# near/near-light-client

Hardware: AMD Instinct MI355X
Metric: Sync/Verify proofs/sec at 1/2/4/8 MI355X + achieved HBM GB/s vs roofline (higher is better)
Workload: dtype u64 (Goldilocks field, integer)

## Files before the change

### near-light-client_amd/csrc/gl32.hpp

```cpp
#pragma once
#include "gl.hpp"
#include "poseidon_blocks.inc"

namespace gl32 {

struct F {
    uint32_t lo, hi;
};

__device__ __forceinline__ F from_u64(uint64_t x) { return F{(uint32_t)x, (uint32_t)(x >> 32)}; }
__device__ __forceinline__ uint64_t to_u64(F x) { return ((uint64_t)x.hi << 32) | x.lo; }

__device__ __forceinline__ F add_w2_eps(uint64_t base, uint32_t w2) {
    uint64_t r;
    uint32_t t;
    asm("v_mad_u64_u32 %[r], vcc, %[w2], -1, %[base]\n\t"
        "v_cndmask_b32_e64 %[t], 0, -1, vcc\n\t"
        "v_mad_u64_u32 %[r], vcc, %[t], 1, %[r]"
        : [r] "=&v"(r), [t] "=&v"(t)
        : [w2] "v"(w2), [base] "v"(base)
        : "vcc");
    return from_u64(r);
}

__device__ __forceinline__ F reduce128(uint32_t w0, uint32_t w1, uint32_t w2, uint32_t w3) {
    uint32_t r0, r1, t0;
    asm("v_sub_co_u32 %[r0], vcc, %[w0], %[w3]\n\t"
        "v_subbrev_co_u32 %[r1], vcc, 0, %[w1], vcc\n\t"
        "v_cndmask_b32_e64 %[t0], 0, -1, vcc\n\t"
        "v_sub_co_u32 %[r0], vcc, %[r0], %[t0]\n\t"
        "v_subbrev_co_u32 %[r1], vcc, 0, %[r1], vcc"
        : [r0] "=&v"(r0), [r1] "=&v"(r1), [t0] "=&v"(t0)
        : [w0] "v"(w0), [w1] "v"(w1), [w3] "v"(w3)
        : "vcc");
    return add_w2_eps(((uint64_t)r1 << 32) | r0, w2);
}

__device__ __forceinline__ uint64_t mad_u64_one(uint32_t a, uint64_t c);

__device__ __forceinline__ F mul(F a, F b) {
#ifdef NLX_GL32_MUL_CARRY_CHAINS
    uint64_t t = (uint64_t)a.lo * b.lo;
    uint64_t m = (uint64_t)a.lo * b.hi;
    uint64_t x = (uint64_t)a.hi * b.hi;
    uint64_t mid;
    uint32_t x1;
    asm("v_mad_u64_u32 %[mid], vcc, %[ah], %[bl], %[m]\n\t"
        "v_addc_co_u32 %[x1], vcc, 0, %[xh], vcc"
        : [mid] "=&v"(mid), [x1] "=v"(x1)
        : [ah] "v"(a.hi), [bl] "v"(b.lo), [m] "v"(m), [xh] "v"((uint32_t)(x >> 32))
        : "vcc");
    uint32_t r0, r1, w1, w2, w3, t0;
    asm("v_add_co_u32 %[w1], vcc, %[th], %[m0]\n\t"
        "v_addc_co_u32 %[w2], vcc, %[x0], %[m1], vcc\n\t"
        "v_addc_co_u32 %[w3], vcc, 0, %[x1], vcc\n\t"
        "v_sub_co_u32 %[r0], vcc, %[w0], %[w3]\n\t"
        "v_subbrev_co_u32 %[r1], vcc, 0, %[w1], vcc\n\t"
        "v_cndmask_b32_e64 %[t0], 0, -1, vcc\n\t"
        "v_sub_co_u32 %[r0], vcc, %[r0], %[t0]\n\t"
        "v_subbrev_co_u32 %[r1], vcc, 0, %[r1], vcc"
        : [r0] "=&v"(r0), [r1] "=&v"(r1), [w1] "=&v"(w1), [w2] "=&v"(w2), [w3] "=&v"(w3), [t0] "=&v"(t0)
        : [w0] "v"((uint32_t)t), [th] "v"((uint32_t)(t >> 32)), [m0] "v"((uint32_t)mid), [x0] "v"((uint32_t)x),
          [m1] "v"((uint32_t)(mid >> 32)), [x1] "v"(x1)
        : "vcc");
    return add_w2_eps(((uint64_t)r1 << 32) | r0, w2);
#else
    const uint64_t p0 = (uint64_t)a.lo * b.lo;
    const uint64_t p1 = (uint64_t)a.lo * b.hi + (p0 >> 32);
    const uint64_t p2 = (uint64_t)a.hi * b.lo + (uint32_t)p1;
    uint64_t p3 = (uint64_t)a.hi * b.hi + (p1 >> 32);
    p3 = mad_u64_one((uint32_t)(p2 >> 32), p3);
    return reduce128((uint32_t)p0, (uint32_t)p2, (uint32_t)p3, (uint32_t)(p3 >> 32));
#endif
}

__device__ __forceinline__ F add_const(F a, uint64_t c) {
    F r;
    uint32_t t;
    asm("v_add_co_u32 %[r0], vcc, %[a0], %[c0]\n\t"
        "v_addc_co_u32 %[r1], vcc, %[a1], %[c1], vcc\n\t"
        "v_cndmask_b32_e64 %[t], 0, -1, vcc\n\t"
        "v_add_co_u32 %[r0], vcc, %[r0], %[t]\n\t"
        "v_addc_co_u32 %[r1], vcc, 0, %[r1], vcc"
        : [r0] "=&v"(r.lo), [r1] "=&v"(r.hi), [t] "=&v"(t)
        : [a0] "v"(a.lo), [a1] "v"(a.hi), [c0] "s"((uint32_t)c), [c1] "v"((uint32_t)(c >> 32))
        : "vcc");
    return r;
}

__device__ __forceinline__ F add_const_v(F a, uint64_t c) {
    F r;
    uint32_t t;
    asm("v_add_co_u32 %[r0], vcc, %[a0], %[c0]\n\t"
        "v_addc_co_u32 %[r1], vcc, %[a1], %[c1], vcc\n\t"
        "v_cndmask_b32_e64 %[t], 0, -1, vcc\n\t"
        "v_add_co_u32 %[r0], vcc, %[r0], %[t]\n\t"
        "v_addc_co_u32 %[r1], vcc, 0, %[r1], vcc"
        : [r0] "=&v"(r.lo), [r1] "=&v"(r.hi), [t] "=&v"(t)
        : [a0] "v"(a.lo), [a1] "v"(a.hi), [c0] "v"((uint32_t)c), [c1] "v"((uint32_t)(c >> 32))
        : "vcc");
    return r;
}

__device__ __forceinline__ F sbox7(F x) {
    F x2 = mul(x, x);
    F x4 = mul(x2, x2);
    F x3 = mul(x, x2);
    return mul(x3, x4);
}

__device__ __forceinline__ F fold_acc(uint64_t al, uint64_t ah) {
    uint64_t t;
    asm("v_mad_u64_u32 %[t], vcc, %[ah1], -1, %[al]" : [t] "=&v"(t) : [ah1] "v"((uint32_t)(ah >> 32)), [al] "v"(al) : "vcc");
    uint32_t r1, m;
    asm("v_add_co_u32 %[r1], vcc, %[t1], %[ah0]\n\t"
        "v_cndmask_b32_e64 %[m], 0, -1, vcc"
        : [r1] "=v"(r1), [m] "=v"(m)
        : [t1] "v"((uint32_t)(t >> 32)), [ah0] "v"((uint32_t)ah)
        : "vcc");
    uint64_t r;
    asm("v_mad_u64_u32 %[r], vcc, %[m], 1, %[base]" : [r] "=&v"(r) : [m] "v"(m), [base] "v"(((uint64_t)r1 << 32) | (uint32_t)t) : "vcc");
    return from_u64(r);
}

__device__ __forceinline__ void mds_layer(F (&s)[12], const uint64_t* __restrict__ rc_next = nullptr) {
    constexpr uint32_t C[12] = {17, 15, 41, 16, 2, 28, 13, 13, 39, 18, 34, 20};
    F o[12];
#pragma unroll
    for (int r = 0; r < 12; r++) {
        uint64_t al = 0, ah = 0;
        if (rc_next) {
            const uint64_t c = rc_next[r];
            al = (uint32_t)c;
            ah = c >> 32;
        }
#pragma unroll
        for (int i = 0; i < 12; i++) {
            al += (uint64_t)s[(i + r) % 12].lo * C[i];
            ah += (uint64_t)s[(i + r) % 12].hi * C[i];
        }
        if (r == 0) {
            al += (uint64_t)s[0].lo * 8u;
            ah += (uint64_t)s[0].hi * 8u;
        }
        o[r] = fold_acc(al, ah);
    }
#pragma unroll
    for (int i = 0; i < 12; i++) s[i] = o[i];
}


typedef int i32x4_t __attribute__((ext_vector_type(4)));
typedef int i32x16_t __attribute__((ext_vector_type(16)));

__device__ __forceinline__ void keep_whole(const i32x16_t& d) { asm volatile("" : : "v"(d)); }

__device__ __forceinline__ i32x4_t mds_a_fragment(uint32_t lane = threadIdx.x & 63) {
    constexpr int C[12] = {17, 15, 41, 16, 2, 28, 13, 13, 39, 18, 34, 20};
    const uint32_t rho = lane & 31, h = lane >> 5;
    const uint32_t g = (rho >> 2) & 1, r = (rho & 3) + 4 * (rho >> 3);
    uint32_t w[4] = {0, 0, 0, 0};
    if (h == g && rho < 24) {
#pragma unroll
        for (int j = 0; j < 12; j++) {
            uint32_t m = 0;
#pragma unroll
            for (int rr = 0; rr < 12; rr++)
                if ((uint32_t)rr == r) m = (uint32_t)C[(j - rr + 12) % 12] + ((rr == 0 && j == 0) ? 8u : 0u);
            w[j >> 2] |= m << (8 * (j & 3));
        }
        w[3] = r == 0 ? 0x00F88080u : 0x00008080u;
    }
    i32x4_t a;
    a.x = (int)w[0]; a.y = (int)w[1]; a.z = (int)w[2]; a.w = (int)w[3];
    return a;
}
constexpr uint32_t MDS_B_BIAS_SLOTS = 0x00808080u;

__device__ __forceinline__ void transpose_bytes4(uint32_t x0, uint32_t x1, uint32_t x2, uint32_t x3, uint32_t (&p)[4]) {
    const uint32_t t01l = __builtin_amdgcn_perm(x1, x0, 0x05010400u), t01h = __builtin_amdgcn_perm(x1, x0, 0x07030602u);
    const uint32_t t23l = __builtin_amdgcn_perm(x3, x2, 0x05010400u), t23h = __builtin_amdgcn_perm(x3, x2, 0x07030602u);
    p[0] = __builtin_amdgcn_perm(t23l, t01l, 0x05040100u);
    p[1] = __builtin_amdgcn_perm(t23l, t01l, 0x07060302u);
    p[2] = __builtin_amdgcn_perm(t23h, t01h, 0x05040100u);
    p[3] = __builtin_amdgcn_perm(t23h, t01h, 0x07060302u);
}
__device__ __forceinline__ uint64_t mad_u64(uint32_t a, uint32_t b, uint64_t c) {
    uint64_t r, sink;
    asm("v_mad_u64_u32 %0, %1, %2, %3, %4" : "=v"(r), "=s"(sink) : "v"(a), "v"(b), "v"(c));
    return r;
}
__device__ __forceinline__ uint64_t mad_u64_sc(uint32_t a, uint32_t b, uint64_t c_uniform) {
    uint64_t r, sink;
    asm("v_mad_u64_u32 %0, %1, %2, %3, %4" : "=v"(r), "=s"(sink) : "v"(a), "v"(b), "s"(c_uniform));
    return r;
}
__device__ __forceinline__ uint64_t mad_u64_one(uint32_t a, uint64_t c) {
    uint64_t r, sink;
    asm("v_mad_u64_u32 %0, %1, %2, 1, %3" : "=v"(r), "=s"(sink) : "v"(a), "v"(c));
    return r;
}
__device__ __forceinline__ F fold_pair(uint64_t t, uint32_t yh, uint32_t k16) {
    uint64_t z, u, sink, sink2;
    asm("v_mad_u64_u32 %0, %1, %2, %3, 0" : "=v"(z), "=s"(sink) : "v"(yh), "v"(k16));
    asm("v_mad_u64_u32 %0, %1, %2, -1, %3" : "=v"(u), "=s"(sink2) : "v"((uint32_t)(z >> 32)), "v"(t));
    uint32_t r1, m;
    asm("v_add_co_u32 %0, vcc, %2, %3\n\t"
        "v_cndmask_b32_e64 %1, 0, -1, vcc"
        : "=v"(r1), "=v"(m)
        : "v"((uint32_t)(u >> 32)), "v"((uint32_t)z)
        : "vcc");
    return from_u64(mad_u64_one(m, ((uint64_t)r1 << 32) | (uint32_t)u));
}

template <int RC>
__device__ __forceinline__ void mds_layer_mfma(F (&s)[12], const i32x4_t a, const uint64_t* __restrict__ rcb) {
    uint32_t k16 = 65536u, bw = MDS_B_BIAS_SLOTS;
    asm("" : "+v"(k16));
    asm("" : "+v"(bw));
    i32x16_t zero;
#pragma unroll
    for (int i = 0; i < 16; i++) zero[i] = 0;
    uint32_t x[2][12], y[2][12];
#pragma unroll
    for (int half = 0; half < 2; half++) {
        uint32_t pl[4][3];
#pragma unroll
        for (int q = 0; q < 3; q++) {
            uint32_t p[4];
            if (half == 0)
                transpose_bytes4(s[4 * q].lo ^ 0x80808080u, s[4 * q + 1].lo ^ 0x80808080u, s[4 * q + 2].lo ^ 0x80808080u,
                                 s[4 * q + 3].lo ^ 0x80808080u, p);
            else
                transpose_bytes4(s[4 * q].hi ^ 0x80808080u, s[4 * q + 1].hi ^ 0x80808080u, s[4 * q + 2].hi ^ 0x80808080u,
                                 s[4 * q + 3].hi ^ 0x80808080u, p);
#pragma unroll
            for (int b = 0; b < 4; b++) pl[b][q] = p[b];
        }
        i32x16_t d[4];
#pragma unroll
        for (int b = 0; b < 4; b++) {
            i32x4_t bf;
            bf.x = (int)pl[b][0]; bf.y = (int)pl[b][1]; bf.z = (int)pl[b][2]; bf.w = (int)bw;
            d[b] = __builtin_amdgcn_mfma_i32_32x32x32_i8(a, bf, zero, 0, 0, 0);
        }
#pragma unroll
        for (int b = 0; b < 4; b++) keep_whole(d[b]);
#pragma unroll
        for (int r = 0; r < 12; r++) {
            x[half][r] = ((uint32_t)d[1][r] << 8) + (uint32_t)d[0][r];
            y[half][r] = ((uint32_t)d[3][r] << 8) + (uint32_t)d[2][r];
        }
        __builtin_amdgcn_sched_barrier(0);
    }
#pragma unroll
    for (int r = 0; r < 12; r++) {
        if (RC == 2 || (RC == 1 && r == 0)) {
            const uint64_t al = mad_u64_one(x[0][r], mad_u64_sc(y[0][r], k16, rcb[r]));
            const uint64_t ah = mad_u64_one(x[1][r], mad_u64_sc(y[1][r], k16, rcb[12 + r]));
            s[r] = fold_acc(al, ah);
        } else {
            const uint64_t t = mad_u64(y[0][r], k16, ((uint64_t)x[1][r] << 32) | x[0][r]);
            s[r] = fold_pair(t, y[1][r], k16);
        }
    }
}

struct BlockOperands {
    i32x4_t a[3];
    i32x16_t seed;
};

template <int G>
__device__ __forceinline__ uint64_t mad_u64_imm(uint32_t a, uint64_t c) {
    uint64_t r, sink;
    asm("v_mad_u64_u32 %0, %1, %2, %3, %4" : "=v"(r), "=s"(sink) : "v"(a), "n"(G), "v"(c));
    return r;
}
__device__ __forceinline__ F fold_pair_x(uint64_t t, uint32_t yh, uint32_t x2, uint32_t k16) {
    uint64_t z, u, sink, sink2;
    asm("v_mad_u64_u32 %0, %1, %2, %3, 0" : "=v"(z), "=s"(sink) : "v"(yh), "v"(k16));
    const uint32_t e = (uint32_t)(z >> 32) + x2;
    asm("v_mad_u64_u32 %0, %1, %2, -1, %3" : "=v"(u), "=s"(sink2) : "v"(e), "v"(t));
    uint32_t r1, m;
    asm("v_add_co_u32 %0, vcc, %2, %3\n\t"
        "v_cndmask_b32_e64 %1, 0, -1, vcc"
        : "=v"(r1), "=v"(m)
        : "v"((uint32_t)(u >> 32)), "v"((uint32_t)z)
        : "vcc");
    return from_u64(mad_u64_one(m, ((uint64_t)r1 << 32) | (uint32_t)u));
}
__device__ __forceinline__ uint64_t mad_u64_sm(uint32_t a, uint32_t m_uniform, uint64_t c) {
    uint64_t r, sink;
    asm("v_mad_u64_u32 %0, %1, %2, %3, %4" : "=v"(r), "=s"(sink) : "v"(a), "s"(m_uniform), "v"(c));
    return r;
}
template <typename RHO>
__device__ __forceinline__ void dot12(const F (&z)[12], const RHO& rho, uint64_t klo, uint64_t khi, uint64_t& al, uint64_t& ah) {
    al = klo;
    ah = khi;
#pragma unroll
    for (int j = 0; j < 12; j++) {
        al = mad_u64_sm(z[j].lo, rho.v[j], al);
        ah = mad_u64_sm(z[j].hi, rho.v[j], ah);
    }
}
struct BlockRho1 { static constexpr uint32_t v[12] = NLX_POSEIDON_BLOCK_RHO1_INIT; };
struct BlockRho2 { static constexpr uint32_t v[12] = NLX_POSEIDON_BLOCK_RHO2_INIT; };

struct BlockSboxes {
    __device__ __forceinline__ F first(F s0) const { return sbox7(s0); }
    __device__ __forceinline__ F inner(int, F w) const { return sbox7(w); }
    __device__ __forceinline__ void before_matrix_pass() const {}
};

template <int GAMMA21, class Sboxes = BlockSboxes>
__device__ __forceinline__ void partial_block3(F (&s)[12], const BlockOperands& op, const uint64_t* __restrict__ kap,
                                               Sboxes sb = Sboxes{}) {
    uint32_t k16 = 65536u;
    asm("" : "+v"(k16));
    s[0] = sb.first(s[0]);
    uint64_t al, ah;
    dot12(s, BlockRho1{}, kap[2], kap[3], al, ah);
    const F u1 = sb.inner(1, fold_acc(al, ah));
    dot12(s, BlockRho2{}, kap[4], kap[5], al, ah);
    al = mad_u64_imm<GAMMA21>(u1.lo, al);
    ah = mad_u64_imm<GAMMA21>(u1.hi, ah);
    const F u2 = sb.inner(2, fold_acc(al, ah));
    sb.before_matrix_pass();
    uint32_t pl[8][3];
#pragma unroll
    for (int half = 0; half < 2; half++)
#pragma unroll
        for (int q = 0; q < 3; q++) {
            uint32_t p[4];
            if (half == 0)
                transpose_bytes4(s[4 * q].lo ^ 0x80808080u, s[4 * q + 1].lo ^ 0x80808080u, s[4 * q + 2].lo ^ 0x80808080u,
                                 s[4 * q + 3].lo ^ 0x80808080u, p);
            else
                transpose_bytes4(s[4 * q].hi ^ 0x80808080u, s[4 * q + 1].hi ^ 0x80808080u, s[4 * q + 2].hi ^ 0x80808080u,
                                 s[4 * q + 3].hi ^ 0x80808080u, p);
#pragma unroll
            for (int b = 0; b < 4; b++) pl[4 * half + b][q] = p[b];
        }
    uint32_t w3[8];
    {
// ... 57 lines not shown
```

### near-light-client_amd/csrc/hash_kernels.hip

```cpp
#include <hip/hip_runtime.h>
#include "poseidon.hpp"
#include "launch.hpp"

namespace nlx {

__global__ __launch_bounds__(256, 4) void k_permute_batch(uint64_t* __restrict__ states, size_t n) {
    const size_t t_raw = (size_t)blockIdx.x * blockDim.x + threadIdx.x;
    const bool live = t_raw < n;
    const size_t t = live ? t_raw : n - 1;
    uint64_t s[12];
    const ulonglong2* src = reinterpret_cast<const ulonglong2*>(states + t * 12);
#pragma unroll
    for (int i = 0; i < 6; i++) {
        ulonglong2 v = src[i];
        s[2 * i] = v.x;
        s[2 * i + 1] = v.y;
    }
    poseidon::permute(s);
    if (!live) return;
    ulonglong2* dst = reinterpret_cast<ulonglong2*>(states + t * 12);
#pragma unroll
    for (int i = 0; i < 6; i++) dst[i] = make_ulonglong2(s[2 * i], s[2 * i + 1]);
}

__device__ __forceinline__ void store_digest(uint64_t* __restrict__ out, size_t idx, const uint64_t (&s)[12]) {
    ulonglong2* dst = reinterpret_cast<ulonglong2*>(out + idx * 4);
    dst[0] = make_ulonglong2(gl::canon(s[0]), gl::canon(s[1]));
    dst[1] = make_ulonglong2(gl::canon(s[2]), gl::canon(s[3]));
}

__global__ __launch_bounds__(256, 4) void k_hash_leaves_rowmajor(const uint64_t* __restrict__ rows, uint32_t row_len,
                                                              size_t n_rows, uint64_t* __restrict__ digests) {
    const size_t row_raw = (size_t)blockIdx.x * blockDim.x + threadIdx.x;
    const bool live = row_raw < n_rows;
    const size_t row = live ? row_raw : n_rows - 1;
    uint64_t s[12];
#pragma unroll
    for (int i = 0; i < 12; i++) s[i] = 0;
    const uint64_t* p = rows + row * (size_t)row_len;
    if (row_len <= 4) {
        for (uint32_t c = 0; c < row_len; c++) {
            uint64_t v = p[c];
            if (c == 0) s[0] = v; else if (c == 1) s[1] = v; else if (c == 2) s[2] = v; else s[3] = v;
        }
        if (live) store_digest(digests, row, s);
        return;
    }
#pragma unroll 1
    for (uint32_t c = 0; c < row_len; c += 8) {
        const uint32_t rem = row_len - c;
#pragma unroll
        for (int j = 0; j < 8; j++)
            if ((uint32_t)j < rem) s[j] = p[c + j];
        poseidon::permute_loose(s);
    }
    if (live) store_digest(digests, row, s);
}

__global__ __launch_bounds__(256, 4) void k_merkle_level(const uint64_t* __restrict__ children,
                                                      uint64_t* __restrict__ parents, size_t n_parents, size_t tree_words) {
    children += (size_t)blockIdx.y * tree_words;
    parents += (size_t)blockIdx.y * tree_words;
    const size_t i_raw = (size_t)blockIdx.x * blockDim.x + threadIdx.x;
    const bool live = i_raw < n_parents;
    const size_t i = live ? i_raw : n_parents - 1;
    const ulonglong2* src = reinterpret_cast<const ulonglong2*>(children + i * 8);
    uint64_t s[12];
#pragma unroll
    for (int k = 0; k < 4; k++) {
        ulonglong2 v = src[k];
        s[2 * k] = v.x;
        s[2 * k + 1] = v.y;
    }
    s[8] = s[9] = s[10] = s[11] = 0;
    poseidon::permute_loose(s);
    if (live) store_digest(parents, i, s);
}

constexpr size_t MERKLE_WIDE_MAX_PARENTS = (size_t)1 << 14;
constexpr unsigned MERKLE_FUSED_MAX_LEVELS = 6;
void launch_merkle_fused(hipStream_t st, const uint64_t* children, size_t n_children, unsigned levels, uint32_t n_trees, size_t tree_words);

void launch_permute_batch(hipStream_t st, uint64_t* d_states, size_t n) {
    if (!n) return;
    hipLaunchKernelGGL(k_permute_batch, dim3((unsigned)((n + 255) / 256)), dim3(256), 0, st, d_states, n);
}

void launch_hash_leaves_rowmajor(hipStream_t st, const uint64_t* d_rows, uint32_t row_len, size_t n_rows,
                                 uint64_t* d_digests) {
    if (!n_rows) return;
    hipLaunchKernelGGL(k_hash_leaves_rowmajor, dim3((unsigned)((n_rows + 255) / 256)), dim3(256), 0, st, d_rows,
                       row_len, n_rows, d_digests);
}

const uint64_t* launch_merkle_levels(hipStream_t st, uint64_t* d_digests, size_t n_leaves, unsigned cap_height, uint32_t n_trees, size_t tree_words) {
    size_t cap = (size_t)1 << cap_height;
    uint64_t* cur = d_digests;
    size_t lvl = n_leaves;
    while (lvl > cap) {
        uint64_t* nxt = cur + lvl * 4;
        size_t half = lvl >> 1;
        if (half <= MERKLE_WIDE_MAX_PARENTS) {
            unsigned K = 0;
            while (K < MERKLE_FUSED_MAX_LEVELS && (lvl >> K) > cap) K++;
            launch_merkle_fused(st, cur, lvl, K, n_trees, tree_words);
            for (unsigned s = 0; s < K; s++) {
                cur += lvl * 4;
                lvl >>= 1;
            }
            continue;
        }
        hipLaunchKernelGGL(k_merkle_level, dim3((unsigned)((half + 255) / 256), n_trees), dim3(256), 0, st, cur, nxt, half, tree_words);
        cur = nxt;
        lvl = half;
    }
    return cur;
}

}

namespace nlx {

constexpr size_t HASH_LEAVES_WIDE_MAX_ROWS = (size_t)1 << 13;

__global__ __launch_bounds__(256, 4) void k_hash_lde_leaves(const uint64_t* __restrict__ lde, size_t col_stride,
                                                         uint32_t n_cols, unsigned log_n, unsigned rate_bits,
                                                         uint64_t* __restrict__ digests, uint32_t batch_cols, size_t tree_words) {
    if (batch_cols) {
        const uint32_t c0 = blockIdx.y * batch_cols;
        lde += (size_t)c0 * col_stride;
        n_cols = n_cols - c0 < batch_cols ? n_cols - c0 : batch_cols;
        digests += (size_t)blockIdx.y * tree_words;
    }
    const size_t pos_raw = (size_t)blockIdx.x * blockDim.x + threadIdx.x;
    const bool live = (pos_raw >> (log_n + rate_bits)) == 0;
    const size_t pos = live ? pos_raw : ((size_t)1 << (log_n + rate_bits)) - 1;
    uint64_t s[12];
#pragma unroll
    for (int i = 0; i < 12; i++) s[i] = 0;
    const uint64_t* p = lde + pos;
    const uint32_t r = (uint32_t)(pos >> log_n), k = (uint32_t)(pos & (((size_t)1 << log_n) - 1));
    const size_t leaf = ((size_t)gl::bitrev32(r, rate_bits) << log_n) + gl::bitrev32(k, log_n);
    if (n_cols <= 4) {
        for (uint32_t c = 0; c < n_cols; c++) {
            uint64_t v = p[(size_t)c * col_stride];
            if (c == 0) s[0] = v; else if (c == 1) s[1] = v; else if (c == 2) s[2] = v; else s[3] = v;
        }
        if (live) store_digest(digests, leaf, s);
        return;
    }
#pragma unroll 1
    for (uint32_t c = 0; c < n_cols; c += 8) {
        const uint32_t rem = n_cols - c;
#pragma unroll
        for (int j = 0; j < 8; j++)
            if ((uint32_t)j < rem) s[j] = p[(size_t)(c + j) * col_stride];
        poseidon::permute_loose(s);
    }
    if (live) store_digest(digests, leaf, s);
}

void launch_hash_lde_leaves_wide(hipStream_t st, const uint64_t* d_lde, size_t col_stride, uint32_t n_cols, unsigned log_n,
                                 unsigned rate_bits, uint64_t* d_digests, uint32_t batch_cols, size_t tree_words);

__global__ __launch_bounds__(256, 4) void k_hash_lde_groups(const uint64_t* __restrict__ lde, size_t col_stride, uint32_t n_cols,
                                                            uint32_t group, unsigned log_L, uint64_t* __restrict__ out) {
    const size_t pos_raw = (size_t)blockIdx.x * blockDim.x + threadIdx.x;
    const bool live = (pos_raw >> log_L) == 0;
    const size_t L = (size_t)1 << log_L, pos = live ? pos_raw : L - 1;
    const uint32_t g = blockIdx.y, c0 = g * group, c1 = c0 + group < n_cols ? c0 + group : n_cols;
    uint64_t s[12];
#pragma unroll
    for (int i = 0; i < 12; i++) s[i] = 0;
    const uint64_t* p = lde + pos;
#pragma unroll 1
    for (uint32_t c = c0; c < c1; c += 8) {
        const uint32_t rem = c1 - c;
#pragma unroll
        for (int j = 0; j < 8; j++)
            if ((uint32_t)j < rem) s[j] = p[(size_t)(c + j) * col_stride];
        poseidon::permute_loose(s);
    }
    if (!live) return;
#pragma unroll
    for (int j = 0; j < 4; j++) out[((size_t)(4 * g + j) << log_L) + pos] = gl::canon(s[j]);
}

void launch_hash_lde_leaves_grouped(hipStream_t st, const uint64_t* d_lde, size_t col_stride, uint32_t n_cols, uint32_t group,
                                    unsigned log_n, unsigned rate_bits, uint64_t* d_group_digests, uint64_t* d_digests) {
    const size_t rows = (size_t)1 << (log_n + rate_bits);
    const uint32_t K = (n_cols + group - 1) / group;
    hipLaunchKernelGGL(k_hash_lde_groups, dim3((unsigned)((rows + 255) / 256), K), dim3(256), 0, st, d_lde, col_stride, n_cols, group,
                       log_n + rate_bits, d_group_digests);
    launch_hash_lde_leaves(st, d_group_digests, rows, 4 * K, log_n, rate_bits, d_digests, 0, 0);
}

void launch_hash_lde_leaves(hipStream_t st, const uint64_t* d_lde, size_t col_stride, uint32_t n_cols,
                            unsigned log_n, unsigned rate_bits, uint64_t* d_digests, uint32_t batch_cols, size_t tree_words) {
    size_t rows = (size_t)1 << (log_n + rate_bits);
    const uint32_t n_batches = batch_cols ? (n_cols + batch_cols - 1) / batch_cols : 1;
    const uint32_t widest = batch_cols && batch_cols < n_cols ? batch_cols : n_cols;
    if (rows * n_batches <= HASH_LEAVES_WIDE_MAX_ROWS && widest > 16) {
        launch_hash_lde_leaves_wide(st, d_lde, col_stride, n_cols, log_n, rate_bits, d_digests, batch_cols, tree_words);
        return;
    }
    hipLaunchKernelGGL(k_hash_lde_leaves, dim3((unsigned)((rows + 255) / 256), n_batches), dim3(256), 0, st, d_lde, col_stride,
                       n_cols, log_n, rate_bits, d_digests, batch_cols, tree_words);
}

}

namespace nlx {

constexpr unsigned WIDE_GROUPS_PER_BLOCK = 16;

__device__ __forceinline__ gl32::F permute_wide(gl32::F x, uint32_t j, volatile uint64_t* slot) {
    constexpr uint32_t C[12] = {17, 15, 41, 16, 2, 28, 13, 13, 39, 18, 34, 20};
    const uint64_t* rc = poseidon::RC_DEV;
    const uint32_t jj = j < 12 ? j : 0;
    const uint32_t diag = j == 0 ? 8u : 0u;
#pragma unroll 1
    for (int r = 0; r < 30; r++) {
        x = gl32::add_const_v(x, rc[r * 12 + jj]);
        const gl32::F x7 = gl32::sbox7(x);
        const bool full = (r < 4) || (r >= 26);
        if (full || j == 0) x = x7;
        volatile uint64_t* sl = slot + (r & 1) * 12;
        if (j < 12) sl[j] = gl32::to_u64(x);
        __builtin_amdgcn_fence(__ATOMIC_RELEASE, "wavefront");
        __builtin_amdgcn_wave_barrier();
        __builtin_amdgcn_fence(__ATOMIC_ACQUIRE, "wavefront");
        uint64_t al = (uint64_t)x.lo * diag, ah = (uint64_t)x.hi * diag, bl = 0, bh = 0;
#pragma unroll
        for (int i = 0; i < 12; i += 2) {
            uint32_t s0 = jj + i, s1 = jj + i + 1;
            s0 = s0 >= 12 ? s0 - 12 : s0;
            s1 = s1 >= 12 ? s1 - 12 : s1;
            const uint64_t v0 = sl[s0], v1 = sl[s1];
            al += (uint64_t)(uint32_t)v0 * C[i];
            ah += (uint64_t)(uint32_t)(v0 >> 32) * C[i];
            bl += (uint64_t)(uint32_t)v1 * C[i + 1];
            bh += (uint64_t)(uint32_t)(v1 >> 32) * C[i + 1];
        }
        x = gl32::fold_acc(al + bl, ah + bh);
    }
    return x;
}

constexpr unsigned FUSED_GROUPS = 32;

__global__ __launch_bounds__(FUSED_GROUPS * 16) void k_merkle_fused(const uint64_t* __restrict__ children, uint64_t* __restrict__ parents0,
                                                                   size_t n_children, unsigned K, size_t tree_words) {
    children += (size_t)blockIdx.y * tree_words;
    parents0 += (size_t)blockIdx.y * tree_words;
    __shared__ uint64_t slots[FUSED_GROUPS * 24];
    __shared__ uint64_t lv[2][FUSED_GROUPS * 2 * 4];
    const uint32_t j = threadIdx.x & 15, g = threadIdx.x >> 4;
    const uint32_t n_own = 1u << K;
    for (uint32_t i = threadIdx.x; i < n_own * 4; i += FUSED_GROUPS * 16) lv[0][i] = children[((size_t)blockIdx.x << K) * 4 + i];
    __syncthreads();
    uint64_t* outp = parents0;
    size_t level_total = n_children;
    for (unsigned s = 1; s <= K; s++) {
        const uint32_t own = n_own >> s;
// ... 101 lines not shown
```

### near-light-client_amd/csrc/poseidon.hpp

```cpp
#pragma once
#include "gl.hpp"
#if defined(__HIP__)
#include "gl32.hpp"
#endif
#include "poseidon_constants.inc"

namespace poseidon {

constexpr int WIDTH = 12;
constexpr int RATE = 8;
constexpr int N_ROUNDS = 30;
constexpr int HALF_FULL = 4;
constexpr int N_PARTIAL = 22;

#if defined(__HIP__)
__constant__ static const uint64_t RC_DEV[360] = NLX_POSEIDON_ROUND_CONSTANTS_INIT;
__constant__ static const uint64_t LAYER_RCB_DEV[31 * 24] = NLX_POSEIDON_LAYER_RCB_INIT;
__constant__ static const uint32_t BLOCK_FRAGMENTS_DEV[NLX_POSEIDON_BLOCK_K * 64 * 4] = NLX_POSEIDON_BLOCK_FRAGMENTS_INIT;
__constant__ static const uint32_t BLOCK_SEED_DEV[16] = NLX_POSEIDON_BLOCK_SEED_INIT;
__constant__ static const uint64_t BLOCK_KAPPA_DEV[NLX_POSEIDON_N_BLOCKS * 2 * NLX_POSEIDON_BLOCK_K] = NLX_POSEIDON_BLOCK_KAPPA_INIT;
static_assert(NLX_POSEIDON_BLOCK_K == 3 && NLX_POSEIDON_BLOCK_DMAX < (1 << 20), "gl32::partial_block3 is written for these");

__device__ __forceinline__ gl32::BlockOperands block_operands(uint32_t lane = threadIdx.x & 63) {
    gl32::BlockOperands op;
#pragma unroll
    for (int p = 0; p < 3; p++) {
        const uint32_t* f = BLOCK_FRAGMENTS_DEV + (p * 64 + lane) * 4;
        op.a[p].x = (int)f[0]; op.a[p].y = (int)f[1]; op.a[p].z = (int)f[2]; op.a[p].w = (int)f[3];
    }
    const uint32_t zero = lane >> 6;
#pragma unroll
    for (int i = 0; i < 16; i++) op.seed[i] = (int)(BLOCK_SEED_DEV[i] + zero);
    return op;
}
#endif
static const uint64_t RC_HOST[360] = NLX_POSEIDON_ROUND_CONSTANTS_INIT;

GL_HD const uint64_t* rc_table() {
#if defined(__HIP_DEVICE_COMPILE__)
    return RC_DEV;
#else
    return RC_HOST;
#endif
}

GL_HD uint64_t sbox7(uint64_t x) {
    uint64_t x2 = gl::mul_loose(x, x);
    uint64_t x4 = gl::mul_loose(x2, x2);
    uint64_t x3 = gl::mul_loose(x, x2);
    return gl::mul_loose(x3, x4);
}

GL_HD uint64_t mds_fold(uint64_t al, uint64_t ah) {
    uint64_t l = al + (ah << 32);
    uint64_t h = (ah >> 32) + (l < al ? 1u : 0u);
    uint64_t t1 = (h << 32) - h;
    uint64_t res = l + t1;
    if (res < t1) res += gl::EPS;
    return res;
}
GL_HD void mds_layer(uint64_t (&s)[12]) {
    constexpr uint32_t C[12] = {17, 15, 41, 16, 2, 28, 13, 13, 39, 18, 34, 20};
    uint32_t lo[12], hi[12];
#pragma unroll
    for (int i = 0; i < 12; i++) {
        lo[i] = (uint32_t)s[i];
        hi[i] = (uint32_t)(s[i] >> 32);
    }
#pragma unroll
    for (int r = 0; r < 12; r++) {
        uint64_t al = 0, ah = 0;
#pragma unroll
        for (int i = 0; i < 12; i++) {
            al += (uint64_t)lo[(i + r) % 12] * C[i];
            ah += (uint64_t)hi[(i + r) % 12] * C[i];
        }
        if (r == 0) {
            al += (uint64_t)lo[0] * 8u;
            ah += (uint64_t)hi[0] * 8u;
        }
        s[r] = mds_fold(al, ah);
    }
}

GL_HD void permute_loose(uint64_t (&s)[12]) {
    const uint64_t* rc = rc_table();
#if defined(__HIP_DEVICE_COMPILE__)
#if defined(NLX_DEBUG)
    if (__builtin_amdgcn_read_exec() != ~0ull) __builtin_trap();
#endif
    const uint64_t* rcb = LAYER_RCB_DEV;
    const gl32::i32x4_t a = gl32::mds_a_fragment();
    const gl32::BlockOperands op = block_operands();
    gl32::F t[12];
#pragma unroll
    for (int i = 0; i < 12; i++) t[i] = gl32::add_const(gl32::from_u64(s[i]), rc[i]);
#pragma unroll 1
    for (int r = 0; r < HALF_FULL; r++) {
#pragma unroll
        for (int i = 0; i < 12; i++) t[i] = gl32::sbox7(t[i]);
        gl32::mds_layer_mfma<2>(t, a, rcb + (r + 1) * 24);
    }
#pragma unroll 1
    for (int b = 0; b < NLX_POSEIDON_N_BLOCKS; b++)
        gl32::partial_block3<NLX_POSEIDON_BLOCK_GAMMA21>(t, op, BLOCK_KAPPA_DEV + b * 6);
    t[0] = gl32::sbox7(t[0]);
    gl32::mds_layer_mfma<2>(t, a, rcb + (HALF_FULL + N_PARTIAL) * 24);
#pragma unroll 1
    for (int r = HALF_FULL + N_PARTIAL; r < N_ROUNDS - 1; r++) {
#pragma unroll
        for (int i = 0; i < 12; i++) t[i] = gl32::sbox7(t[i]);
        gl32::mds_layer_mfma<2>(t, a, rcb + (r + 1) * 24);
    }
#pragma unroll
    for (int i = 0; i < 12; i++) t[i] = gl32::sbox7(t[i]);
    gl32::mds_layer_mfma<0>(t, a, rcb);
#pragma unroll
    for (int i = 0; i < 12; i++) s[i] = gl32::to_u64(t[i]);
#else
#pragma unroll 1
    for (int r = 0; r < HALF_FULL; r++) {
        for (int i = 0; i < 12; i++) s[i] = sbox7(gl::add_loose(s[i], rc[r * 12 + i]));
        mds_layer(s);
    }
    for (int r = HALF_FULL; r < HALF_FULL + N_PARTIAL; r++) {
        for (int i = 0; i < 12; i++) s[i] = gl::add_loose(s[i], rc[r * 12 + i]);
        s[0] = sbox7(s[0]);
        mds_layer(s);
    }
    for (int r = HALF_FULL + N_PARTIAL; r < N_ROUNDS; r++) {
        for (int i = 0; i < 12; i++) s[i] = sbox7(gl::add_loose(s[i], rc[r * 12 + i]));
        mds_layer(s);
    }
#endif
}

GL_HD void permute(uint64_t (&s)[12]) {
    permute_loose(s);
#pragma unroll
    for (int i = 0; i < 12; i++) s[i] = gl::canon(s[i]);
}

}
```

### near-light-client_amd/csrc/prover_kernels.hip

```cpp
#include <hip/hip_runtime.h>
#include "gl.hpp"
#include "poseidon.hpp"
#include "poseidon_fast_constants.inc"
#include "prover.hpp"

namespace nlx {

__constant__ static const uint64_t FAST_FIRST[12] = NLX_POSEIDON_FAST_FIRST_RC_INIT;
__constant__ static const uint64_t FAST_RC[22] = NLX_POSEIDON_FAST_RC_INIT;
__constant__ static const uint64_t FAST_VS[22][11] = NLX_POSEIDON_FAST_VS_INIT;
__constant__ static const uint64_t FAST_W[22][11] = NLX_POSEIDON_FAST_W_HATS_INIT;
__constant__ static const uint64_t FAST_INIT[11][11] = NLX_POSEIDON_FAST_INITIAL_MATRIX_INIT;

__device__ __forceinline__ uint64_t root_pow(const uint64_t* __restrict__ half_table, uint32_t e, uint32_t half) {
    return e < half ? half_table[e] : gl::P - half_table[e - half];
}

__global__ __launch_bounds__(256) void k_zs_row_products(ZsParams p) {
    const size_t i = (size_t)blockIdx.x * blockDim.x + threadIdx.x;
    const size_t n = (size_t)1 << p.log_n;
    if (i >= n) return;
    const uint64_t x = root_pow(p.w_n_table, (uint32_t)i, (uint32_t)(n >> 1));
    constexpr int MAXQ = 10;
    uint64_t num[2 * MAXQ], den[2 * MAXQ];
// ... 1051 lines not shown
    if (pos >> log_L) return;
    const size_t L = (size_t)1 << log_L;
    const uint32_t lo = blockIdx.y * per_slice, hi = lo + per_slice;
    gl::Ext s0, s1;
    fri_column_sums(p, pos, L, lo, hi, s0, s1);
    uint64_t* dst = part + (((size_t)blockIdx.y << log_L) + pos) * 4;
    dst[0] = s0.a; dst[1] = s0.b; dst[2] = s1.a; dst[3] = s1.b;
}
__global__ __launch_bounds__(256) void k_fri_combine_finish(FriCombineParams p, uint32_t slices, const uint64_t* __restrict__ part) {
    const size_t pos = (size_t)blockIdx.x * blockDim.x + threadIdx.x;
    const unsigned log_L = p.log_n + p.rate_bits;
    if (pos >> log_L) return;
    const size_t n = (size_t)1 << p.log_n;
    gl::Ext s0{0, 0}, s1{0, 0};
    for (uint32_t sl = 0; sl < slices; sl++) {
        const uint64_t* src = part + (((size_t)sl << log_L) + pos) * 4;
        s0 = gl::add(s0, gl::Ext{src[0], src[1]});
        s1 = gl::add(s1, gl::Ext{src[2], src[3]});
    }
    const uint32_t r = (uint32_t)(pos >> p.log_n), k = (uint32_t)(pos & (n - 1));
    const uint64_t x = gl::mul(p.coset_base[r], root_pow(p.w_n_table, k, (uint32_t)(n >> 1)));
    const gl::Ext zeta{p.zeta[0], p.zeta[1]}, gzeta{p.gzeta[0], p.gzeta[1]};
    const gl::Ext d0 = gl::sub(gl::ext(x), zeta), d1 = gl::sub(gl::ext(x), gzeta);
    const gl::Ext inv01 = gl::inv(gl::mul(d0, d1));
    const gl::Ext i0 = gl::mul(inv01, d1), i1 = gl::mul(inv01, d0);
    gl::Ext q0 = gl::mul(gl::sub(s0, gl::Ext{p.c0[0], p.c0[1]}), i0);
    q0 = gl::mul(q0, gl::Ext{p.alpha_nz[0], p.alpha_nz[1]});
    const gl::Ext q1 = gl::mul(gl::sub(s1, gl::Ext{p.c1[0], p.c1[1]}), i1);
    const gl::Ext res = gl::add(q0, q1);
    reinterpret_cast<ulonglong2*>(p.out)[pos] = make_ulonglong2(res.a, res.b);
}

uint32_t fri_combine_slices(const FriCombineParams& p) {
    const size_t L = (size_t)1 << (p.log_n + p.rate_bits);
    uint32_t cols = 0;
    for (int o = 0; o < FRI_VIEWS; o++) cols += p.n_cols[o];
    if (L >= ((size_t)1 << 15) || cols < 256) return 1;
    uint32_t want = (uint32_t)((((size_t)1 << 17) + L - 1) / L);
    const uint32_t max_slices = cols / 64 ? cols / 64 : 1;
    if (want > max_slices) want = max_slices;
    return want > 64 ? 64 : want;
}
size_t fri_combine_scratch_words(const FriCombineParams& p) {
    const uint32_t s = fri_combine_slices(p);
    return s > 1 ? ((size_t)s << (p.log_n + p.rate_bits)) * 4 : 0;
}
void launch_fri_combine(hipStream_t st, const FriCombineParams& p, uint64_t* scratch) {
    const size_t L = (size_t)1 << (p.log_n + p.rate_bits);
    const uint32_t slices = scratch ? fri_combine_slices(p) : 1;
    if (slices <= 1) {
        hipLaunchKernelGGL(k_fri_combine, dim3((unsigned)((L + 255) / 256)), dim3(256), 0, st, p);
        return;
    }
    uint32_t cols = 0;
    for (int o = 0; o < FRI_VIEWS; o++) cols += p.n_cols[o];
    const uint32_t per_slice = (cols + slices - 1) / slices;
    hipLaunchKernelGGL(k_fri_combine_partial, dim3((unsigned)((L + 255) / 256), slices), dim3(256), 0, st, p, per_slice, scratch);
    hipLaunchKernelGGL(k_fri_combine_finish, dim3((unsigned)((L + 255) / 256)), dim3(256), 0, st, p, slices, scratch);
}

template <int ARITY_BITS>
__global__ __launch_bounds__(256, 4) void k_fri_leaves(const uint64_t* __restrict__ values, unsigned log_n,
                                                    unsigned rate_bits, uint64_t* __restrict__ digests) {
    constexpr int ARITY = 1 << ARITY_BITS;
    const unsigned log_np = log_n - ARITY_BITS;
    const size_t jp_raw = (size_t)blockIdx.x * blockDim.x + threadIdx.x;
    const bool live = (jp_raw >> (log_np + rate_bits)) == 0;
    const size_t jp = live ? jp_raw : ((size_t)1 << (log_np + rate_bits)) - 1;
    const size_t np = (size_t)1 << log_np, n = (size_t)1 << log_n;
    const uint32_t r = (uint32_t)(jp >> log_np), kp = (uint32_t)(jp & (np - 1));
    const ulonglong2* v = reinterpret_cast<const ulonglong2*>(values) + ((size_t)r * n + kp);
    uint64_t s[12];
#pragma unroll
    for (int i = 0; i < 12; i++) s[i] = 0;
    for (int m0 = 0; m0 < ARITY; m0 += 4) {
#pragma unroll
        for (int t = 0; t < 4; t++) {
            const int m = m0 + t;
            const int mm = (int)(__brev((unsigned)m) >> (32 - ARITY_BITS));
            const ulonglong2 e = v[(size_t)mm * np];
            s[2 * t] = e.x;
            s[2 * t + 1] = e.y;
        }
        poseidon::permute_loose(s);
    }
    if (!live) return;
    const size_t leaf = ((size_t)gl::bitrev32(r, rate_bits) << log_np) + gl::bitrev32(kp, log_np);
    ulonglong2* dst = reinterpret_cast<ulonglong2*>(digests + leaf * 4);
    dst[0] = make_ulonglong2(gl::canon(s[0]), gl::canon(s[1]));
    dst[1] = make_ulonglong2(gl::canon(s[2]), gl::canon(s[3]));
}
void launch_fri_leaves(hipStream_t st, const uint64_t* d_values, unsigned log_n, unsigned rate_bits,
                       unsigned arity_bits, uint64_t* d_digests) {
    const size_t leaves = (size_t)1 << (log_n - arity_bits + rate_bits);
    const unsigned blocks = (unsigned)((leaves + 255) / 256);
    if (arity_bits == 4) hipLaunchKernelGGL(k_fri_leaves<4>, dim3(blocks), dim3(256), 0, st, d_values, log_n, rate_bits, d_digests);
    else if (arity_bits == 3) hipLaunchKernelGGL(k_fri_leaves<3>, dim3(blocks), dim3(256), 0, st, d_values, log_n, rate_bits, d_digests);
    else if (arity_bits == 2) hipLaunchKernelGGL(k_fri_leaves<2>, dim3(blocks), dim3(256), 0, st, d_values, log_n, rate_bits, d_digests);
}

template <int ARITY_BITS>
__global__ __launch_bounds__(256) void k_fri_fold(const uint64_t* __restrict__ values, uint64_t* __restrict__ out,
                                                  unsigned log_n, unsigned rate_bits, uint64_t beta_a, uint64_t beta_b,
                                                  uint64_t shift_inv, const uint64_t* __restrict__ w_L_inv_table,
                                                  const uint64_t* __restrict__ w_A_inv_pows, uint64_t arity_inv) {
    constexpr int ARITY = 1 << ARITY_BITS;
    const unsigned log_np = log_n - ARITY_BITS;
    const unsigned log_L = log_n + rate_bits;
    const size_t jp_raw = (size_t)blockIdx.x * blockDim.x + threadIdx.x;
    const bool live = (jp_raw >> (log_np + rate_bits)) == 0;
    const size_t jp = live ? jp_raw : ((size_t)1 << (log_np + rate_bits)) - 1;
    const size_t np = (size_t)1 << log_np, n = (size_t)1 << log_n;
    const uint32_t r = (uint32_t)(jp >> log_np), kp = (uint32_t)(jp & (np - 1));
    const ulonglong2* v = reinterpret_cast<const ulonglong2*>(values) + ((size_t)r * n + kp);
    gl::Ext a[ARITY];
#pragma unroll
    for (int mm = 0; mm < ARITY; mm++) {
        const ulonglong2 e = v[(size_t)mm * np];
        a[mm] = gl::Ext{e.x, e.y};
    }
    const uint32_t ip = (kp << rate_bits) + r;
    const uint64_t x_inv = gl::mul(shift_inv, root_pow(w_L_inv_table, ip, 1u << (log_L - 1)));
    const gl::Ext bx = gl::mul(gl::Ext{beta_a, beta_b}, x_inv);
    gl::Ext res{0, 0};
#pragma unroll 1
    for (int t = ARITY - 1; t >= 0; t--) {
        gl::Ext c{0, 0};
#pragma unroll
        for (int mm = 0; mm < ARITY; mm++) c = gl::add(c, gl::mul(a[mm], w_A_inv_pows[(t * mm) & (ARITY - 1)]));
        res = gl::add(gl::mul(res, bx), c);
    }
    res = gl::mul(res, arity_inv);
    reinterpret_cast<ulonglong2*>(out)[jp] = make_ulonglong2(res.a, res.b);
}
void launch_fri_fold(hipStream_t st, const uint64_t* d_values, uint64_t* d_out, unsigned log_n, unsigned rate_bits,
                     unsigned arity_bits, const uint64_t beta[2], uint64_t shift_inv, const uint64_t* d_w_L_inv_table,
                     const uint64_t* d_w_A_inv_pows) {
    const size_t outs = (size_t)1 << (log_n - arity_bits + rate_bits);
    const unsigned blocks = (unsigned)((outs + 255) / 256);
    const uint64_t ainv = gl::inv((uint64_t)1 << arity_bits);
    if (arity_bits == 4) hipLaunchKernelGGL(k_fri_fold<4>, dim3(blocks), dim3(256), 0, st, d_values, d_out, log_n, rate_bits, beta[0], beta[1], shift_inv, d_w_L_inv_table, d_w_A_inv_pows, ainv);
    else if (arity_bits == 3) hipLaunchKernelGGL(k_fri_fold<3>, dim3(blocks), dim3(256), 0, st, d_values, d_out, log_n, rate_bits, beta[0], beta[1], shift_inv, d_w_L_inv_table, d_w_A_inv_pows, ainv);
    else if (arity_bits == 2) hipLaunchKernelGGL(k_fri_fold<2>, dim3(blocks), dim3(256), 0, st, d_values, d_out, log_n, rate_bits, beta[0], beta[1], shift_inv, d_w_L_inv_table, d_w_A_inv_pows, ainv);
}

__global__ void k_fri_final_coeffs(const uint64_t* __restrict__ values, unsigned log_n, unsigned rate_bits,
                                   uint64_t shift_inv, uint64_t w_L_inv, uint64_t L_inv, uint64_t* __restrict__ out,
                                   uint32_t n_out) {
    const uint32_t j = blockIdx.x * blockDim.x + threadIdx.x;
    if (j >= n_out) return;
    const unsigned log_L = log_n + rate_bits;
    const size_t L = (size_t)1 << log_L, n = (size_t)1 << log_n;
    const uint64_t wj = gl::pow(w_L_inv, j);
    uint64_t wij = 1;
    gl::Ext acc{0, 0};
    for (size_t i = 0; i < L; i++) {
        const size_t pos = ((i & ((1u << rate_bits) - 1)) * n) + (i >> rate_bits);
        const gl::Ext v{values[2 * pos], values[2 * pos + 1]};
        acc = gl::add(acc, gl::mul(v, wij));
        wij = gl::mul(wij, wj);
    }
    acc = gl::mul(acc, gl::mul(gl::pow(shift_inv, j), L_inv));
    out[2 * j] = acc.a;
    out[2 * j + 1] = acc.b;
}
void launch_fri_final_coeffs(hipStream_t st, const uint64_t* d_values, unsigned log_n, unsigned rate_bits,
                             uint64_t shift, uint64_t* d_out, uint32_t n_out) {
// ... 87 lines not shown
```

Before: 22.59.

## Specialize Poseidon sponge permutations for zero capacity and partial outputs

Adds a permute_sponge variant that knows how the state enters and leaves each absorb step. When the capacity is zero, the first-round S-box on the capacity lanes is replaced by precomputed constants. When the capacity is already seeded, the round-constant add is folded into the previous permutation's last MDS. The final MDS layer computes only the 4 output lanes actually consumed (the digest head, or the capacity for the next absorb). All leaf, row and Merkle hashing kernels are rewired to use it, trading extra branching and code size for fewer field multiplies and MFMA post-processing per permutation.

```diff
diff --git a/near-light-client_amd/csrc/gl32.hpp b/near-light-client_amd/csrc/gl32.hpp
--- a/near-light-client_amd/csrc/gl32.hpp
+++ b/near-light-client_amd/csrc/gl32.hpp
@@ -88,6 +88,20 @@
     return r;
 }
 
+__device__ __forceinline__ F add_const_sc(F a, uint64_t c_uniform) {
+    uint64_t t, sink;
+    asm("v_mad_u64_u32 %0, %1, %2, 1, %3" : "=v"(t), "=s"(sink) : "v"(a.lo), "s"(c_uniform));
+    uint32_t r1, m;
+    asm("v_add_co_u32 %[r1], vcc, %[t1], %[a1]\n\t"
+        "v_cndmask_b32_e64 %[m], 0, -1, vcc"
+        : [r1] "=v"(r1), [m] "=v"(m)
+        : [t1] "v"((uint32_t)(t >> 32)), [a1] "v"(a.hi)
+        : "vcc");
+    uint64_t r;
+    asm("v_mad_u64_u32 %[r], vcc, %[m], 1, %[base]" : [r] "=&v"(r) : [m] "v"(m), [base] "v"(((uint64_t)r1 << 32) | (uint32_t)t) : "vcc");
+    return from_u64(r);
+}
+
 __device__ __forceinline__ F add_const_v(F a, uint64_t c) {
     F r;
     uint32_t t;
@@ -213,8 +227,12 @@
     return from_u64(mad_u64_one(m, ((uint64_t)r1 << 32) | (uint32_t)u));
 }
 
+enum : uint32_t { OUT_ALL = 0, OUT_HEAD4 = 1, OUT_CAP4 = 2 };
+
 template <int RC>
-__device__ __forceinline__ void mds_layer_mfma(F (&s)[12], const i32x4_t a, const uint64_t* __restrict__ rcb) {
+__device__ __forceinline__ void mds_layer_mfma(F (&s)[12], const i32x4_t a, const uint64_t* __restrict__ rcb,
+                                               const uint32_t sel = OUT_ALL) {
+    const bool all = RC != 0 || sel == OUT_ALL;
     uint32_t k16 = 65536u, bw = MDS_B_BIAS_SLOTS;
     asm("" : "+v"(k16));
     asm("" : "+v"(bw));
@@ -246,22 +264,42 @@
         }
 #pragma unroll
         for (int b = 0; b < 4; b++) keep_whole(d[b]);
+        auto planes = [&](int r0, int r1) {
+#pragma unroll
+            for (int r = r0; r < r1; r++) {
+                x[half][r] = ((uint32_t)d[1][r] << 8) + (uint32_t)d[0][r];
+                y[half][r] = ((uint32_t)d[3][r] << 8) + (uint32_t)d[2][r];
+            }
+        };
+        if (all) planes(0, 12);
+        else if (sel == OUT_HEAD4) planes(0, 4);
+        else planes(8, 12);
+        __builtin_amdgcn_sched_barrier(0);
+    }
+    auto seeded = [&](int r) {
+        const uint64_t al = mad_u64_one(x[0][r], mad_u64_sc(y[0][r], k16, rcb[r]));
+        const uint64_t ah = mad_u64_one(x[1][r], mad_u64_sc(y[1][r], k16, rcb[12 + r]));
+        s[r] = fold_acc(al, ah);
+    };
+    auto plain = [&](int r) {
+        const uint64_t t = mad_u64(y[0][r], k16, ((uint64_t)x[1][r] << 32) | x[0][r]);
+        s[r] = fold_pair(t, y[1][r], k16);
+    };
+    if (all) {
 #pragma unroll
         for (int r = 0; r < 12; r++) {
-            x[half][r] = ((uint32_t)d[1][r] << 8) + (uint32_t)d[0][r];
-            y[half][r] = ((uint32_t)d[3][r] << 8) + (uint32_t)d[2][r];
-        }
-        __builtin_amdgcn_sched_barrier(0);
-    }
-#pragma unroll
-    for (int r = 0; r < 12; r++) {
-        if (RC == 2 || (RC == 1 && r == 0)) {
-            const uint64_t al = mad_u64_one(x[0][r], mad_u64_sc(y[0][r], k16, rcb[r]));
-            const uint64_t ah = mad_u64_one(x[1][r], mad_u64_sc(y[1][r], k16, rcb[12 + r]));
-            s[r] = fold_acc(al, ah);
+            if (RC == 2 || (RC == 1 && r == 0)) seeded(r);
+            else plain(r);
+        }
+    } else {
+#pragma unroll
+        for (int r = 0; r < 12; r++) s[r] = F{__builtin_nondeterministic_value(0u), __builtin_nondeterministic_value(0u)};
+        if (sel == OUT_HEAD4) {
+#pragma unroll
+            for (int r = 0; r < 4; r++) plain(r);
         } else {
-            const uint64_t t = mad_u64(y[0][r], k16, ((uint64_t)x[1][r] << 32) | x[0][r]);
-            s[r] = fold_pair(t, y[1][r], k16);
+#pragma unroll
+            for (int r = 8; r < 12; r++) seeded(r);
         }
     }
 }
diff --git a/near-light-client_amd/csrc/hash_kernels.hip b/near-light-client_amd/csrc/hash_kernels.hip
--- a/near-light-client_amd/csrc/hash_kernels.hip
+++ b/near-light-client_amd/csrc/hash_kernels.hip
@@ -46,13 +46,16 @@
         if (live) store_digest(digests, row, s);
         return;
     }
+    uint32_t in = poseidon::IN_CAP_ZERO;
 #pragma unroll 1
     for (uint32_t c = 0; c < row_len; c += 8) {
         const uint32_t rem = row_len - c;
 #pragma unroll
         for (int j = 0; j < 8; j++)
             if ((uint32_t)j < rem) s[j] = p[c + j];
-        poseidon::permute_loose(s);
+        const uint32_t out = poseidon::sponge_out(rem > 8 ? rem - 8 : 0);
+        poseidon::permute_sponge(s, in, out);
+        in = poseidon::sponge_in(out);
     }
     if (live) store_digest(digests, row, s);
 }
@@ -73,7 +76,7 @@
         s[2 * k + 1] = v.y;
     }
     s[8] = s[9] = s[10] = s[11] = 0;
-    poseidon::permute_loose(s);
+    poseidon::permute_sponge(s, poseidon::IN_CAP_ZERO, gl32::OUT_HEAD4);
     if (live) store_digest(parents, i, s);
 }
 
@@ -149,13 +152,16 @@
         if (live) store_digest(digests, leaf, s);
         return;
     }
+    uint32_t in = poseidon::IN_CAP_ZERO;
 #pragma unroll 1
     for (uint32_t c = 0; c < n_cols; c += 8) {
         const uint32_t rem = n_cols - c;
 #pragma unroll
         for (int j = 0; j < 8; j++)
             if ((uint32_t)j < rem) s[j] = p[(size_t)(c + j) * col_stride];
-        poseidon::permute_loose(s);
+        const uint32_t out = poseidon::sponge_out(rem > 8 ? rem - 8 : 0);
+        poseidon::permute_sponge(s, in, out);
+        in = poseidon::sponge_in(out);
     }
     if (live) store_digest(digests, leaf, s);
 }
@@ -173,13 +179,16 @@
 #pragma unroll
     for (int i = 0; i < 12; i++) s[i] = 0;
     const uint64_t* p = lde + pos;
+    uint32_t in = poseidon::IN_CAP_ZERO;
 #pragma unroll 1
     for (uint32_t c = c0; c < c1; c += 8) {
         const uint32_t rem = c1 - c;
 #pragma unroll
         for (int j = 0; j < 8; j++)
             if ((uint32_t)j < rem) s[j] = p[(size_t)(c + j) * col_stride];
-        poseidon::permute_loose(s);
+        const uint32_t out = poseidon::sponge_out(rem > 8 ? rem - 8 : 0);
+        poseidon::permute_sponge(s, in, out);
+        in = poseidon::sponge_in(out);
     }
     if (!live) return;
 #pragma unroll
diff --git a/near-light-client_amd/csrc/poseidon.hpp b/near-light-client_amd/csrc/poseidon.hpp
--- a/near-light-client_amd/csrc/poseidon.hpp
+++ b/near-light-client_amd/csrc/poseidon.hpp
@@ -4,6 +4,7 @@
 #include "gl32.hpp"
 #endif
 #include "poseidon_constants.inc"
+#include "poseidon_tails.inc"
 
 namespace poseidon {
 
@@ -20,6 +21,10 @@
 __constant__ static const uint32_t BLOCK_SEED_DEV[16] = NLX_POSEIDON_BLOCK_SEED_INIT;
 __constant__ static const uint64_t BLOCK_KAPPA_DEV[NLX_POSEIDON_N_BLOCKS * 2 * NLX_POSEIDON_BLOCK_K] = NLX_POSEIDON_BLOCK_KAPPA_INIT;
 static_assert(NLX_POSEIDON_BLOCK_K == 3 && NLX_POSEIDON_BLOCK_DMAX < (1 << 20), "gl32::partial_block3 is written for these");
+__constant__ static const uint64_t TAIL_RCB_DEV[24] = NLX_POSEIDON_TAIL_RCB_INIT;
+__constant__ static const uint64_t SBOX_RC0_CAP_DEV[4] = NLX_POSEIDON_SBOX_RC0_CAP_INIT;
+
+enum : uint32_t { IN_PLAIN = 0, IN_CAP_SEEDED = 1, IN_CAP_ZERO = 2 };
 
 __device__ __forceinline__ gl32::BlockOperands block_operands(uint32_t lane = threadIdx.x & 63) {
     gl32::BlockOperands op;
@@ -83,9 +88,13 @@
     }
 }
 
-GL_HD void permute_loose(uint64_t (&s)[12]) {
-    const uint64_t* rc = rc_table();
-#if defined(__HIP_DEVICE_COMPILE__)
+#if defined(__HIP__)
+__device__ __forceinline__ void permute_sponge(uint64_t (&s)[12], uint32_t in, uint32_t out) {
+#ifdef NLX_POSEIDON_FULL_TAILS
+    in = IN_PLAIN;
+    out = gl32::OUT_ALL;
+#endif
+    const uint64_t* rc = RC_DEV;
 #if defined(NLX_DEBUG)
     if (__builtin_amdgcn_read_exec() != ~0ull) __builtin_trap();
 #endif
@@ -94,11 +103,27 @@
     const gl32::BlockOperands op = block_operands();
     gl32::F t[12];
 #pragma unroll
-    for (int i = 0; i < 12; i++) t[i] = gl32::add_const(gl32::from_u64(s[i]), rc[i]);
+    for (int i = 0; i < RATE; i++) t[i] = gl32::add_const_sc(gl32::from_u64(s[i]), rc[i]);
+    if (in == IN_PLAIN) {
+#pragma unroll
+        for (int i = RATE; i < 12; i++) t[i] = gl32::add_const_sc(gl32::from_u64(s[i]), rc[i]);
+    } else {
+#pragma unroll
+        for (int i = RATE; i < 12; i++) t[i] = gl32::from_u64(s[i]);
+    }
 #pragma unroll 1
     for (int r = 0; r < HALF_FULL; r++) {
 #pragma unroll
-        for (int i = 0; i < 12; i++) t[i] = gl32::sbox7(t[i]);
+        for (int i = 0; i < RATE; i++) t[i] = gl32::sbox7(t[i]);
+        if (r == 0 && in == IN_CAP_ZERO) {
+            const uint64_t* sb = SBOX_RC0_CAP_DEV;
+            asm volatile("" : "+s"(sb));
+#pragma unroll
+            for (int i = RATE; i < 12; i++) t[i] = gl32::from_u64(sb[i - RATE]);
+        } else {
+#pragma unroll
+            for (int i = RATE; i < 12; i++) t[i] = gl32::sbox7(t[i]);
+        }
         gl32::mds_layer_mfma<2>(t, a, rcb + (r + 1) * 24);
     }
 #pragma unroll 1
@@ -114,10 +139,22 @@
     }
 #pragma unroll
     for (int i = 0; i < 12; i++) t[i] = gl32::sbox7(t[i]);
-    gl32::mds_layer_mfma<0>(t, a, rcb);
+    gl32::mds_layer_mfma<0>(t, a, TAIL_RCB_DEV, out);
 #pragma unroll
     for (int i = 0; i < 12; i++) s[i] = gl32::to_u64(t[i]);
+}
+
+__device__ __forceinline__ uint32_t sponge_out(uint32_t left) {
+    return left == 0 ? gl32::OUT_HEAD4 : left >= (uint32_t)RATE ? gl32::OUT_CAP4 : gl32::OUT_ALL;
+}
+__device__ __forceinline__ uint32_t sponge_in(uint32_t prev_out) { return prev_out == gl32::OUT_CAP4 ? IN_CAP_SEEDED : IN_PLAIN; }
+#endif
+
+GL_HD void permute_loose(uint64_t (&s)[12]) {
+#if defined(__HIP_DEVICE_COMPILE__)
+    permute_sponge(s, IN_PLAIN, gl32::OUT_ALL);
 #else
+    const uint64_t* rc = rc_table();
 #pragma unroll 1
     for (int r = 0; r < HALF_FULL; r++) {
         for (int i = 0; i < 12; i++) s[i] = sbox7(gl::add_loose(s[i], rc[r * 12 + i]));
diff --git a/near-light-client_amd/csrc/poseidon_tails.inc b/near-light-client_amd/csrc/poseidon_tails.inc
--- /dev/null
+++ b/near-light-client_amd/csrc/poseidon_tails.inc
@@ -0,0 +1,2 @@
+#define NLX_POSEIDON_TAIL_RCB_INIT { 0x00000000ull, 0x00000000ull, 0x00000000ull, 0x00000000ull, 0x00000000ull, 0x00000000ull, 0x00000000ull, 0x00000000ull, 0xb0c44426ull, 0xbf337bffull, 0x9da578a1ull, 0x25db2c76ull, 0x00000000ull, 0x00000000ull, 0x00000000ull, 0x00000000ull, 0x00000000ull, 0x00000000ull, 0x00000000ull, 0x00000000ull, 0xcdc4a239ull, 0x277fa208ull, 0xe17653a2ull, 0xc54302f2ull }
+#define NLX_POSEIDON_SBOX_RC0_CAP_INIT { 0xc70fa963a6d76d43ull, 0x8046358185c6e230ull, 0x6e54c050fb2a6ae5ull, 0xb1742ab4a8c81453ull }
diff --git a/near-light-client_amd/csrc/prover_kernels.hip b/near-light-client_amd/csrc/prover_kernels.hip
--- a/near-light-client_amd/csrc/prover_kernels.hip
+++ b/near-light-client_amd/csrc/prover_kernels.hip
@@ -1157,7 +1157,8 @@
             s[2 * t] = e.x;
             s[2 * t + 1] = e.y;
         }
-        poseidon::permute_loose(s);
+        poseidon::permute_sponge(s, m0 == 0 ? poseidon::IN_CAP_ZERO : poseidon::IN_CAP_SEEDED,
+                                 m0 + 4 < ARITY ? gl32::OUT_CAP4 : gl32::OUT_HEAD4);
     }
     if (!live) return;
     const size_t leaf = ((size_t)gl::bitrev32(r, rate_bits) << log_np) + gl::bitrev32(kp, log_np);
```

After: 22.79 (median of 6 runs). Within noise of the previous version (+0.9%).
